# dbolya/yolact

Measured on AMD Instinct MI355X. Metric: images/sec (550x550, batch 8 per GPU), YOLACT yolact_resnet50 forward + Detect (Fast NMS), higher is better.
Workload: dtype f32 (fp32 in / fp32 accumulate / fp32 out; 92 % of the GEMM time on fp16x2 tiles = every fp32 operand as two fp16 pieces by round to nearest (22 significant bits + 2 signs: exact for ~2/3 of all fp32 values, one fp32 ulp otherwise), 3 exact piece products per product on the fp16 matrix pipe; measure

## Files before the change

### include/yolact_amd.h

```cpp
#ifndef YOLACT_AMD_H
#define YOLACT_AMD_H
#include <stddef.h>
#include <stdint.h>

#ifdef __cplusplus
extern "C" {
#endif

#define YMI_ABI_VERSION 9

#define YMI_EFORMAT (-4)
#define YMI_EUNSUPPORTED (-5)

enum { YMI_ACT_NONE = 0, YMI_ACT_RELU = 1, YMI_ACT_LEAKY01 = 2, YMI_ACT_TANH = 3, YMI_ACT_SIGMOID = 4 };
enum { YMI_RES_NONE = 0, YMI_RES_ADD = 1, YMI_RES_BILINEAR = 2 };

typedef struct {
  int32_t n0, n1;
  int32_t act;
  int32_t row_stride;
  int64_t batch_stride;
  float *ptr;
} ymi_conv_seg;

// ... 535 lines not shown
  int64_t ws_bytes;
  int32_t B, H, W, Cout, ldg, _pad0;
} ymi_stem_wgrad_desc;
int ymi_stem_wgrad_nhwc_f32(const ymi_stem_wgrad_desc *d, void *stream);

int ymi_maxpool_fwd_nhwc_f32(const float *x, float *y, int B, int H, int W, int C, void *stream);
int ymi_maxpool_bwd_nhwc_f32(const float *x, const float *dy, float *dx, int B, int H, int W, int C, void *stream);

typedef struct ymi_stem_desc {
  const float *x;
  float *y;
  int32_t B, H, W, cout_pad;
  const void *w_h2;
  const float *scale_h2, *bias;
  float *y_amax;
  int32_t kpad, _pad0;
} ymi_stem_desc;
int ymi_stem_pool_f32(const ymi_stem_desc *d, void *stream);

typedef struct ymi_chain_desc {
  const float *x, *res;
  float *y, *z;
  const void *w_a_h2, *w_b_h2;
  const float *scale_a_h2, *bias_a, *scale_b_h2, *bias_b;
  const float *x_amax;
  float *y_amax, *z_amax;
  int64_t M;
  int32_t ldx, res_ld, ldy, ldz;
  int32_t k_a, n_a, n_b;
  int32_t cout_pad_a, cout_pad_b;
  int32_t act_a, act_b, _pad0;
  const float *res_amax;
  float gain_a, bias_max_a;
} ymi_chain_desc;
int ymi_pointwise_chain_f32(const ymi_chain_desc *d, void *stream);

typedef struct ymi_stage_exit_desc {
  ymi_chain_desc chain;
  int32_t B, H, W, y_stride;
} ymi_stage_exit_desc;
int ymi_stage_exit_chain_f32(const ymi_stage_exit_desc *d, void *stream);

enum { YMI_OP_NOP = 0, YMI_OP_CONV = 1, YMI_OP_WINO = 2, YMI_OP_DCN = 3, YMI_OP_CHAIN = 4, YMI_OP_STEM = 5, YMI_OP_INPUT = 6,
       YMI_OP_BILINEAR = 7, YMI_OP_MAXPOOL = 8, YMI_OP_BILINEAR_ADD = 9, YMI_OP_RECORD = 10, YMI_OP_WAIT = 11, YMI_OP_MEMSET = 12,
       YMI_OP_STAGE_EXIT = 13 };
enum { YMI_SEC_NONE = 0, YMI_SEC_BACKBONE = 1, YMI_SEC_FPN = 2, YMI_SEC_PROTO = 3, YMI_SEC_HEADS = 4 };
typedef struct ymi_plan_op {
  int32_t kind;
  int32_t stream;
  int32_t section;
  int32_t _pad;
  const void *desc;
  void *p[3];
  int64_t i[8];
  double f[2];
} ymi_plan_op;
int ymi_event_create(void **ev);
int ymi_event_destroy(void *ev);
int ymi_plan_run(const ymi_plan_op *ops, int first, int last, void *stream_a, void *stream_b, void *const *events, int overlap,
                 int skip_sections, int32_t *failed_op);

enum {
  YMI_WS_WINO_V = 1,
  YMI_WS_WINO_M = 2,
  YMI_WS_SPLITK = 3,
  YMI_WS_MASK_IOU = 4,
// ... 78 lines not shown
```

### yolact_amd/_lib.py

```python
from __future__ import annotations

import ctypes as C
import os

_HERE = os.path.dirname(os.path.abspath(__file__))
LIB_PATH = os.path.join(_HERE, 'libyolact_amd.so')

ABI_VERSION = 9

ACT_NONE, ACT_RELU, ACT_LEAKY01, ACT_TANH, ACT_SIGMOID = 0, 1, 2, 3, 4
RES_NONE, RES_ADD, RES_BILINEAR = 0, 1, 2
TILE_AUTO, TILE_128x128, TILE_128x64, TILE_64x64, TILE_128x32, TILE_64x128 = 0, 1, 2, 3, 4, 5
TILE_32x32_K4, TILE_64x32_K2, TILE_32x64_K2 = 6, 7, 8
TILE_64x64_S3, TILE_64x64_S4, TILE_64x128_S3, TILE_128x64_S3, TILE_32x32_K4_S4, TILE_64x32_K2_S3, TILE_32x64_K2_S3 = range(9, 16)
TILE_NAMES = {1: '128x128', 2: '128x64', 3: '64x64', 4: '128x32', 5: '64x128', 6: '32x32k4', 7: '64x32k2', 8: '32x64k2',
              9: '64x64s3', 10: '64x64s4', 11: '64x128s3', 12: '128x64s3', 13: '32x32k4s4', 14: '64x32k2s3', 15: '32x64k2s3',
              16: '128x128w8', 17: '256x128w8', 18: '128x256w8', 19: '128x128s3', 20: '128x128w8s3', 21: '256x128w8s3',
              22: '128x128w8s4'}
TILE_128x128_W8, TILE_256x128_W8, TILE_128x256_W8 = 16, 17, 18
TILE_128x128_S3, TILE_128x128_W8_S3, TILE_256x128_W8_S3, TILE_128x128_W8_S4 = 19, 20, 21, 22
TILE_WG_128x256 = 23
TILE_X3 = 32
X3_BASE_TILES = (1, 2, 3, 5, 6, 7, 8, 9, 11, 12, 16, 17, 19, 20, 21, 22)
for _t in X3_BASE_TILES:
# ... 241 lines not shown
                ('out_class', C.c_void_p), ('out_coef', C.c_void_p), ('out_prior', C.c_void_p), ('out_rec', C.c_void_p)]


class DetectGreedyWs(C.Structure):
    _fields_ = [('box_scale', C.c_float), ('_pad0', C.c_int32), ('ws', C.c_void_p)]


class JpegInfo(C.Structure):
    _fields_ = [('width', C.c_int32), ('height', C.c_int32), ('ncomp', C.c_int32), ('progressive', C.c_int32),
                ('orientation', C.c_int32), ('color', C.c_int32), ('out_width', C.c_int32), ('out_height', C.c_int32),
                ('hs', C.c_int32 * 3), ('vs', C.c_int32 * 3), ('hf', C.c_int32 * 3), ('vf', C.c_int32 * 3),
                ('bw', C.c_int32 * 3), ('bh', C.c_int32 * 3), ('dw', C.c_int32 * 3), ('dh', C.c_int32 * 3),
                ('coef_count', C.c_int64), ('plane_bytes', C.c_int64)]


class JpegEncDesc(C.Structure):
    _fields_ = [('img', C.c_void_p), ('h', C.c_int32), ('w', C.c_int32), ('row_stride', C.c_int64), ('quality', C.c_int32),
                ('subsampling', C.c_int32), ('out', C.c_void_p), ('out_capacity', C.c_int64), ('out_len', C.c_void_p),
                ('ws', C.c_void_p)]


JPEG_SUB_444, JPEG_SUB_420 = 0, 2
JPEG_HEADER_BYTES = 623


class ChainDesc(C.Structure):
    _fields_ = [('x', C.c_void_p), ('res', C.c_void_p), ('y', C.c_void_p), ('z', C.c_void_p),
                ('w_a_h2', C.c_void_p), ('w_b_h2', C.c_void_p),
                ('scale_a_h2', C.c_void_p), ('bias_a', C.c_void_p), ('scale_b_h2', C.c_void_p), ('bias_b', C.c_void_p),
                ('x_amax', C.c_void_p), ('y_amax', C.c_void_p), ('z_amax', C.c_void_p),
                ('M', C.c_int64), ('ldx', C.c_int32), ('res_ld', C.c_int32), ('ldy', C.c_int32), ('ldz', C.c_int32),
                ('k_a', C.c_int32), ('n_a', C.c_int32), ('n_b', C.c_int32), ('cout_pad_a', C.c_int32), ('cout_pad_b', C.c_int32),
                ('act_a', C.c_int32), ('act_b', C.c_int32), ('_pad0', C.c_int32),
                ('res_amax', C.c_void_p), ('gain_a', C.c_float), ('bias_max_a', C.c_float)]


class StageExitDesc(C.Structure):
    _fields_ = [('chain', ChainDesc), ('B', C.c_int32), ('H', C.c_int32), ('W', C.c_int32), ('y_stride', C.c_int32)]


class StemDesc(C.Structure):
    _fields_ = [('x', C.c_void_p), ('y', C.c_void_p), ('B', C.c_int32), ('H', C.c_int32), ('W', C.c_int32), ('cout_pad', C.c_int32),
                ('w_h2', C.c_void_p), ('scale_h2', C.c_void_p), ('bias', C.c_void_p), ('y_amax', C.c_void_p),
                ('kpad', C.c_int32), ('_pad0', C.c_int32)]


class PlanOp(C.Structure):
    _fields_ = [('kind', C.c_int32), ('stream', C.c_int32), ('section', C.c_int32), ('_pad', C.c_int32), ('desc', C.c_void_p),
                ('p', C.c_void_p * 3), ('i', C.c_int64 * 8), ('f', C.c_double * 2)]


(OP_NOP, OP_CONV, OP_WINO, OP_DCN, OP_CHAIN, OP_STEM, OP_INPUT, OP_BILINEAR, OP_MAXPOOL, OP_BILINEAR_ADD, OP_RECORD, OP_WAIT,
 OP_MEMSET, OP_STAGE_EXIT) = range(14)
SEC_NONE, SEC_BACKBONE, SEC_FPN, SEC_PROTO, SEC_HEADS = range(5)


class MaskIouShape(C.Structure):
    _fields_ = [('A', C.c_int32), ('B', C.c_int32), ('n', C.c_int64)]


class ApMatchDesc(C.Structure):
    _fields_ = [('cls', C.c_void_p), ('box_score', C.c_void_p), ('mask_score', C.c_void_p), ('box_iou', C.c_void_p),
                ('mask_iou', C.c_void_p), ('crowd_box_iou', C.c_void_p), ('crowd_mask_iou', C.c_void_p), ('gt_cls', C.c_void_p),
                ('crowd_cls', C.c_void_p), ('rec_key', C.c_void_p), ('rec_score', C.c_void_p), ('rec_flags', C.c_void_p),
                ('gt_count', C.c_void_p), ('base', C.c_int64), ('cap', C.c_int64),
                ('N', C.c_int32), ('G', C.c_int32), ('Gc', C.c_int32), ('num_classes', C.c_int32)]

# ... 160 lines not shown
```

### yolact_amd/csrc/chain.hip

```cpp
#include "gemm_h2.h"
#include <type_traits>

int ymi_internal_prof_begin(double flops, int tile, int kind, hipStream_t s);
void ymi_internal_prof_end(int idx, hipStream_t s);

namespace {

using namespace ymi_h2;

typedef unsigned u32x4 __attribute__((ext_vector_type(4)));

constexpr int K1 = 64, N1 = 256, PX = 32, NW = 8;
constexpr int RS1 = 2 * K1 + 16;
constexpr int RS2 = 2 * N1 + 16;
constexpr int A1_PLANE = PX * RS1, A2_PLANE = PX * RS2;
constexpr int A1_BUF = 2 * A1_PLANE, A2_BUF = 2 * A2_PLANE;
constexpr int OFF_A1 = 0, OFF_A2 = OFF_A1 + 2 * A1_BUF, OFF_SC = OFF_A2 + 2 * A2_BUF, OFF_EP = OFF_SC + 2 * (2 * NW * 4),
              CH_LDS = OFF_EP + NW * 2 * 4 * 32;
constexpr int OFF_EP2 = CH_LDS, OFF_WL = OFF_EP2 + NW * 2 * 4 * 32, CH_LDS_X = OFF_WL + 128 * N1 * 2;
static_assert(CH_LDS_X <= 160 * 1024, "LDS of a CU");

struct ChainParams {
  const float *x, *res, *x_amax;
  const void *wa, *wb;
  const float *sa, *ba, *sb, *bb;
  float *y, *z, *y_amax, *z_amax;
  int M, ldx, res_ld, ldy, ldz, act_a, act_b;
  unsigned wa_plane, wb_plane;
};
struct ChainParamsX : ChainParams {
  unsigned long long mag_w, mag_h;
  int H, W, y_stride;
};

template <int N2>
__global__ __launch_bounds__(64 * NW) void chain_h2_k(const std::conditional_t<N2 == 128, ChainParamsX, ChainParams> p) {
#if defined(__HIP_DEVICE_COMPILE__)
  constexpr int NT = N2 / 64;
  constexpr bool EXIT = N2 == 128;
  __shared__ __attribute__((aligned(16))) char lds[EXIT ? CH_LDS_X : CH_LDS];
  const int t = threadIdx.x, lane = t & 63, wave = __builtin_amdgcn_readfirstlane(t >> 6);
  const int lr = lane & 15, g = lane >> 4;
  const int q2 = wave & 3, i2 = wave >> 2;
  float sA, invA;
  ymi_h2_scale(ymi_amax_read(p.x_amax), sA, invA);
  const ymi_amax_pre apre_y = ymi_amax_prefetch(p.y_amax);
  const ymi_amax_pre apre_z = ymi_amax_prefetch(p.z_amax);
  const bool two = p.z != nullptr;

  f16x8 w3h[2][2], w3l[2][2], w1h[NT][8], w1l[EXIT ? 1 : NT][EXIT ? 1 : 8];
#pragma unroll
  for (int j = 0; j < 2; ++j)
#pragma unroll
    for (int c = 0; c < 2; ++c) {
      const char *src = reinterpret_cast<const char *>(p.wa) + (size_t)(32 * wave + 16 * j + lr) * (2 * K1) + c * 64 + g * 16;
      w3h[j][c] = *reinterpret_cast<const f16x8 *>(src);
      w3l[j][c] = *reinterpret_cast<const f16x8 *>(src + p.wa_plane);
    }
#pragma unroll
  for (int tt = 0; tt < NT; ++tt)
#pragma unroll
    for (int c = 0; c < 8; ++c) {
      const f16x8 z8 = {0, 0, 0, 0, 0, 0, 0, 0};
      const char *src = reinterpret_cast<const char *>(p.wb) + (size_t)(16 * NT * q2 + 16 * tt + lr) * (2 * N1) + c * 64 + g * 16;
      w1h[tt][c] = two ? *reinterpret_cast<const f16x8 *>(src) : z8;
      if constexpr (!EXIT) w1l[tt][c] = two ? *reinterpret_cast<const f16x8 *>(src + p.wb_plane) : z8;
    }
  if constexpr (EXIT) {
#pragma unroll
    for (int k = 0; k < 8; ++k) {
      const int c = t >> 6;
      const char *src = reinterpret_cast<const char *>(p.wb) + p.wb_plane + (size_t)(16 * k + lr) * (2 * N1) + c * 64 + g * 16;
      const f16x8 z8 = {0, 0, 0, 0, 0, 0, 0, 0};
      *reinterpret_cast<f16x8 *>(lds + OFF_WL + ((k * 8 + c) * 64 + lane) * 16) = two ? *reinterpret_cast<const f16x8 *>(src) : z8;
    }
  }
  if (lr == 0) {
#pragma unroll
    for (int j = 0; j < 2; ++j) {
      const int n = 32 * wave + 16 * j + 4 * g;
      f32x4 sc, bi;
#pragma unroll
      for (int e = 0; e < 4; ++e) { sc[e] = p.sa[n + e] * invA; bi[e] = p.ba ? p.ba[n + e] : 0.f; }
      *reinterpret_cast<f32x4 *>(lds + OFF_EP + ((wave * 2 + j) * 4 + g) * 32) = sc;
      *reinterpret_cast<f32x4 *>(lds + OFF_EP + ((wave * 2 + j) * 4 + g) * 32 + 16) = bi;
    }
  }
  f32x4 sc1 = {1.f, 1.f, 1.f, 1.f}, bi1 = {0.f, 0.f, 0.f, 0.f};
  if constexpr (EXIT) {
    if (lr == 0) {
#pragma unroll
      for (int tt = 0; tt < NT; ++tt) {
        const int n = 16 * NT * q2 + 16 * tt + 4 * g;
        f32x4 sc = sc1, bi = bi1;
        if (two) {
#pragma unroll
          for (int e = 0; e < 4; ++e) { sc[e] = p.sb[n + e]; bi[e] = p.bb ? p.bb[n + e] : 0.f; }
        }
        *reinterpret_cast<f32x4 *>(lds + OFF_EP2 + ((wave * 2 + tt) * 4 + g) * 32) = sc;
        *reinterpret_cast<f32x4 *>(lds + OFF_EP2 + ((wave * 2 + tt) * 4 + g) * 32 + 16) = bi;
      }
    }
  } else if (two) {
#pragma unroll
    for (int e = 0; e < 4; ++e) { sc1[e] = p.sb[16 * q2 + 4 * g + e]; bi1[e] = p.bb ? p.bb[16 * q2 + 4 * g + e] : 0.f; }
  }
  const float slope_a = ymi_act_slope(p.act_a);
  const float slope_b = ymi_act_slope(p.act_b);

  const int ntiles = (p.M + PX - 1) / PX;
  const __amdgpu_buffer_rsrc_t xrs = buf_rsrc(p.x, (unsigned)p.M * (unsigned)p.ldx * 4u);
  const __amdgpu_buffer_rsrc_t rrs = buf_rsrc(p.res ? p.res : p.x, p.res ? (int)((unsigned)p.M * (unsigned)p.res_ld * 4u) : 0);
  const __amdgpu_buffer_rsrc_t yrs = buf_rsrc(p.y, (unsigned)p.M * (unsigned)p.ldy * 4u);
  const __amdgpu_buffer_rsrc_t zrs = buf_rsrc(p.z ? p.z : p.y, p.z ? (int)((unsigned)p.M * (unsigned)p.ldz * 4u) : 0);
  const int xp = t >> 4, xc = t & 15;
  auto load_x = [&](int tile) {
    const int m = tile * PX + xp;
    const unsigned off = (tile < ntiles && m < p.M) ? (unsigned)(m * p.ldx + 4 * xc) * 4u : OOB;
    return __builtin_bit_cast(f32x4, __builtin_amdgcn_raw_buffer_load_b128(xrs, off, 0, 0));
  };
  auto load_res = [&](int tile, f32x4 (&r)[2][2]) {
#pragma unroll
    for (int i = 0; i < 2; ++i) {
      const int m = tile * PX + 16 * i + lr;
      const unsigned off = (tile < ntiles && m < p.M) ? (unsigned)(m * p.res_ld + 32 * wave + 4 * g) * 4u : OOB;
#pragma unroll
      for (int j = 0; j < 2; ++j) r[i][j] = __builtin_bit_cast(f32x4, __builtin_amdgcn_raw_buffer_load_b128(rrs, off + 64u * j, 0, 0));
    }
  };

  float am_y = 0.f, am_z = 0.f;
  f32x4 xv;
  const int grid = (int)gridDim.x;
  auto iteration = [&](const int tile, auto buf_c, f32x4 (&rv)[2][2], f32x4 (&rn)[2][2]) {
    constexpr int BUF = decltype(buf_c)::value;
    char *const a1 = lds + OFF_A1 + BUF * A1_BUF;
    char *const a2w = lds + OFF_A2 + BUF * A2_BUF;
    const char *const a2r = lds + OFF_A2 + (BUF ^ 1) * A2_BUF;
    float *const scw = reinterpret_cast<float *>(lds + OFF_SC) + BUF * (2 * NW);
    const float *const scr = reinterpret_cast<const float *>(lds + OFF_SC) + (BUF ^ 1) * (2 * NW);
    {
      const f32x4 v = xv * sA;
      f16x4 h4, l4;
#pragma unroll
      for (int e = 0; e < 4; ++e) {
        const _Float16 h = (_Float16)v[e];
        h4[e] = h;
        l4[e] = (_Float16)(v[e] - (float)h);
      }
      char *dst = a1 + xp * RS1 + xc * 8;
      *reinterpret_cast<f16x4 *>(dst) = h4;
      *reinterpret_cast<f16x4 *>(dst + A1_PLANE) = l4;
    }
    xv = load_x(tile + grid);
    load_res(tile + grid, rn);
    YMI_BARRIER();
    if (two) {
      f32x4 tot[NT];
#pragma unroll
      for (int tt = 0; tt < NT; ++tt) tot[tt] = f32x4{0.f, 0.f, 0.f, 0.f};
#pragma unroll
      for (int c0 = 0; c0 < 8; c0 += 2) {
        f16x8 xh[2], xl[2];
        f32x4 a2[2][NT];
#pragma unroll
        for (int u = 0; u < 2; ++u) {
          xh[u] = *reinterpret_cast<const f16x8 *>(a2r + (16 * i2 + lr) * RS2 + (c0 + u) * 64 + g * 16);
          xl[u] = *reinterpret_cast<const f16x8 *>(a2r + A2_PLANE + (16 * i2 + lr) * RS2 + (c0 + u) * 64 + g * 16);
#pragma unroll
          for (int tt = 0; tt < NT; ++tt) a2[u][tt] = f32x4{0.f, 0.f, 0.f, 0.f};
        }
        if constexpr (EXIT) {
          f16x8 wl[2][NT];
#pragma unroll
          for (int u = 0; u < 2; ++u)
#pragma unroll
            for (int tt = 0; tt < NT; ++tt)
              wl[u][tt] = *reinterpret_cast<const f16x8 *>(lds + OFF_WL + ((((NT * q2 + tt) * 8) + c0 + u) * 64 + lane) * 16);
#pragma unroll
          for (int pr = 0; pr < 3; ++pr)
#pragma unroll
            for (int u = 0; u < 2; ++u)
#pragma unroll
              for (int tt = 0; tt < NT; ++tt)
                a2[u][tt] = ymi_mfma16(pr == 0 ? wl[u][tt] : w1h[tt][c0 + u], pr == 1 ? xl[u] : xh[u], a2[u][tt]);
        } else {
#pragma unroll
          for (int pr = 0; pr < 3; ++pr)
// ... 29 lines not shown
    f32x4 acc[2][2];
#pragma unroll
    for (int i = 0; i < 2; ++i)
#pragma unroll
      for (int j = 0; j < 2; ++j) acc[i][j] = f32x4{0.f, 0.f, 0.f, 0.f};
#pragma unroll
    for (int c = 0; c < 2; ++c) {
      f16x8 xh[2], xl[2];
#pragma unroll
      for (int i = 0; i < 2; ++i) {
        xh[i] = *reinterpret_cast<const f16x8 *>(a1 + (16 * i + lr) * RS1 + c * 64 + g * 16);
        xl[i] = *reinterpret_cast<const f16x8 *>(a1 + A1_PLANE + (16 * i + lr) * RS1 + c * 64 + g * 16);
      }
#pragma unroll
      for (int pr = 0; pr < 3; ++pr)
#pragma unroll
        for (int i = 0; i < 2; ++i)
#pragma unroll
          for (int j = 0; j < 2; ++j)
            acc[i][j] = ymi_mfma16(pr == 0 ? w3l[j][c] : w3h[j][c], pr == 1 ? xl[i] : xh[i], acc[i][j]);
    }
#pragma unroll
    for (int i = 0; i < 2; ++i) {
      const int m = tile * PX + 16 * i + lr;
      const bool ok = m < p.M;
      bool keep = ok;
      if constexpr (EXIT) {
        const unsigned r = (unsigned)(((unsigned long long)(unsigned)m * p.mag_w) >> 32);
        const unsigned w = (unsigned)m - r * (unsigned)p.W;
        const unsigned h = r - (unsigned)(((unsigned long long)r * p.mag_h) >> 32) * (unsigned)p.H;
        keep = ok && (p.y_stride == 1 || ((h | w) & 1u) == 0);
      }
      const unsigned yoff = keep ? (unsigned)(m * p.ldy + 32 * wave + 4 * g) * 4u : OOB;
      float tm = 0.f;
#pragma unroll
      for (int j = 0; j < 2; ++j) {
        const f32x4 sc3 = *reinterpret_cast<const f32x4 *>(lds + OFF_EP + ((wave * 2 + j) * 4 + g) * 32);
        const f32x4 bi3 = *reinterpret_cast<const f32x4 *>(lds + OFF_EP + ((wave * 2 + j) * 4 + g) * 32 + 16);
        f32x4 v = acc[i][j] * sc3 + bi3 + rv[i][j];
#pragma unroll
        for (int e = 0; e < 4; ++e) v[e] = fmaxf(v[e], slope_a * v[e]);
        if (!ok) v = f32x4{0.f, 0.f, 0.f, 0.f};
        acc[i][j] = v;
        tm = fmaxf(tm, ymi_absmax4(v));
        __builtin_amdgcn_raw_buffer_store_b128(__builtin_bit_cast(u32x4, v), yrs, yoff + 64u * j, 0, 0);
      }
      am_y = fmaxf(am_y, tm);
      if (two) {
        const unsigned tmb = ymi_wave_umax63(__builtin_bit_cast(unsigned, tm));
        float sT, invT;
        ymi_h2_scale(__builtin_bit_cast(float, (unsigned)__builtin_amdgcn_readlane((int)tmb, 63)), sT, invT);
#pragma unroll
        for (int j = 0; j < 2; ++j) {
          const f32x4 v = acc[i][j] * sT;
          f16x4 h4, l4;
#pragma unroll
          for (int e = 0; e < 4; ++e) {
            const _Float16 h = (_Float16)v[e];
            h4[e] = h;
            l4[e] = (_Float16)(v[e] - (float)h);
          }
          char *dst = a2w + (16 * i + lr) * RS2 + (32 * wave + 16 * j + 4 * g) * 2;
          *reinterpret_cast<f16x4 *>(dst) = h4;
          *reinterpret_cast<f16x4 *>(dst + A2_PLANE) = l4;
        }
        if (lane == 0) scw[i * NW + wave] = invT;
      }
    }
  };
  int tile = blockIdx.x;
  f32x4 ra[2][2], rb[2][2];
  xv = load_x(tile);
  load_res(tile, ra);
  for (; tile < ntiles + (two ? grid : 0); tile += 2 * grid) {
    iteration(tile, std::integral_constant<int, 0>{}, ra, rb);
    iteration(tile + grid, std::integral_constant<int, 1>{}, rb, ra);
  }
  if (p.y_amax) ymi_amax_finish(apre_y, am_y);
  if (two && p.z_amax) ymi_amax_finish(apre_z, am_z);
#endif
}

}

int ymi_internal_chain2(const ymi_chain_desc *d, hipStream_t s);

extern "C" int ymi_pointwise_chain_f32(const ymi_chain_desc *d, void *stream) {
  if (!d) return YMI_ENULL;
  if (!d->x || !d->w_a_h2 || !d->scale_a_h2 || !d->y || !d->x_amax) return YMI_ENULL;
  if (d->z && (!d->w_b_h2 || !d->scale_b_h2)) return YMI_ENULL;
  const bool wide = d->k_a == 128 || d->k_a == 256;
  if (d->M <= 0 || (!wide && (d->k_a != K1 || d->n_a != N1 || (d->z && d->n_b != 64)))) return YMI_EARG;
  if (wide && (d->n_a != 4 * d->k_a || (d->z && d->n_b != d->k_a))) return YMI_EARG;
  if (d->act_a < 0 || d->act_a > YMI_ACT_LEAKY01 || d->act_b < 0 || d->act_b > YMI_ACT_LEAKY01) return YMI_EARG;
  if (d->ldx < d->k_a || d->ldy < d->n_a || (d->z && d->ldz < d->n_b) || (d->res && d->res_ld < d->n_a)) return YMI_ESHAPE;
  if ((d->ldx | d->ldy | d->ldz | d->res_ld) & 3) return YMI_ESHAPE;
  if ((((uintptr_t)d->x) | ((uintptr_t)d->y) | ((uintptr_t)d->z) | ((uintptr_t)d->res) | ((uintptr_t)d->w_a_h2) | ((uintptr_t)d->w_b_h2)) & 15)
    return YMI_ESHAPE;
  if (d->M * (int64_t)(d->ldy > d->res_ld ? d->ldy : d->res_ld) >= (1LL << 29) || d->M * (int64_t)d->ldx >= (1LL << 29)) return YMI_ESHAPE;
  if (wide) return ymi_internal_chain2(d, (hipStream_t)stream);
  if (d->cout_pad_a < N1 || (d->z && d->cout_pad_b < 64)) return YMI_ESHAPE;
  ChainParams p;
  p.x = d->x; p.res = d->res; p.x_amax = d->x_amax; p.wa = d->w_a_h2; p.wb = d->w_b_h2;
  p.sa = d->scale_a_h2; p.ba = d->bias_a; p.sb = d->scale_b_h2; p.bb = d->bias_b;
  p.y = d->y; p.z = d->z; p.y_amax = d->y_amax; p.z_amax = d->z_amax;
  p.M = (int)d->M; p.ldx = d->ldx; p.res_ld = d->res_ld; p.ldy = d->ldy; p.ldz = d->ldz; p.act_a = d->act_a; p.act_b = d->act_b;
  p.wa_plane = (unsigned)((long)d->cout_pad_a * K1 * 2); p.wb_plane = (unsigned)((long)d->cout_pad_b * N1 * 2);
  hipStream_t s = (hipStream_t)stream;
  const int pr = ymi_internal_prof_begin(2.0 * (double)d->M * K1 * N1, YMI_TILE_H2 | YMI_TILE_64x64, 13, s);
  int dev = 0, cus = 256;
  hipGetDevice(&dev);
  hipDeviceGetAttribute(&cus, hipDeviceAttributeMultiprocessorCount, dev);
  const long ntiles = (d->M + PX - 1) / PX;
  hipLaunchKernelGGL(chain_h2_k<64>, dim3((unsigned)(ntiles < cus ? ntiles : cus)), dim3(64 * NW), 0, s, p);
  const int rc = ymi_launch_status();
  ymi_internal_prof_end(pr, s);
  if (rc == YMI_OK && d->z) {
    const int p2 = ymi_internal_prof_begin(2.0 * (double)d->M * N1 * 64, YMI_TILE_H2 | YMI_TILE_64x64, 12, s);
    ymi_internal_prof_end(p2, s);
  }
  return rc;
}

extern "C" int ymi_stage_exit_chain_f32(const ymi_stage_exit_desc *e, void *stream) {
  if (!e) return YMI_ENULL;
  const ymi_chain_desc *d = &e->chain;
  if (!d->x || !d->w_a_h2 || !d->scale_a_h2 || !d->y || !d->x_amax || !d->z || !d->w_b_h2 || !d->scale_b_h2) return YMI_ENULL;
  if (d->k_a != K1 || d->n_a != N1 || d->n_b != 128 || (e->y_stride != 1 && e->y_stride != 2)) return YMI_EARG;
  if (d->M <= 0 || e->B <= 0 || e->H <= 0 || e->W <= 0 || d->M != (int64_t)e->B * e->H * e->W) return YMI_EARG;
  if (d->act_a < 0 || d->act_a > YMI_ACT_LEAKY01 || d->act_b < 0 || d->act_b > YMI_ACT_LEAKY01) return YMI_EARG;
  if (d->ldx < K1 || d->ldy < N1 || d->ldz < 128 || (d->res && d->res_ld < N1)) return YMI_ESHAPE;
  if ((d->ldx | d->ldy | d->ldz | d->res_ld) & 3) return YMI_ESHAPE;
  if ((((uintptr_t)d->x) | ((uintptr_t)d->y) | ((uintptr_t)d->z) | ((uintptr_t)d->res) | ((uintptr_t)d->w_a_h2) | ((uintptr_t)d->w_b_h2)) & 15)
    return YMI_ESHAPE;
  const int64_t ldmax = d->ldy > d->res_ld ? (d->ldy > d->ldz ? d->ldy : d->ldz) : (d->res_ld > d->ldz ? d->res_ld : d->ldz);
  if (d->M * ldmax >= (1LL << 29) || d->M * (int64_t)d->ldx >= (1LL << 29)) return YMI_ESHAPE;
  if (d->cout_pad_a < N1 || d->cout_pad_b < 128) return YMI_ESHAPE;
  if (d->M * (int64_t)(e->H > e->W ? e->H : e->W) >= (1LL << 32)) return YMI_ESHAPE;
  ChainParamsX p;
  p.x = d->x; p.res = d->res; p.x_amax = d->x_amax; p.wa = d->w_a_h2; p.wb = d->w_b_h2;
  p.sa = d->scale_a_h2; p.ba = d->bias_a; p.sb = d->scale_b_h2; p.bb = d->bias_b;
  p.y = d->y; p.z = d->z; p.y_amax = d->y_amax; p.z_amax = d->z_amax;
  p.M = (int)d->M; p.ldx = d->ldx; p.res_ld = d->res_ld; p.ldy = d->ldy; p.ldz = d->ldz; p.act_a = d->act_a; p.act_b = d->act_b;
  p.wa_plane = (unsigned)((long)d->cout_pad_a * K1 * 2); p.wb_plane = (unsigned)((long)d->cout_pad_b * N1 * 2);
  p.H = e->H; p.W = e->W; p.y_stride = e->y_stride;
  p.mag_w = ((1ULL << 32) + (unsigned)e->W - 1) / (unsigned)e->W;
  p.mag_h = ((1ULL << 32) + (unsigned)e->H - 1) / (unsigned)e->H;
  hipStream_t s = (hipStream_t)stream;
  const int pr = ymi_internal_prof_begin(2.0 * (double)d->M * K1 * N1, YMI_TILE_H2 | YMI_TILE_64x64, 13, s);
  int dev = 0, cus = 256;
  hipGetDevice(&dev);
  hipDeviceGetAttribute(&cus, hipDeviceAttributeMultiprocessorCount, dev);
  const long ntiles = (d->M + PX - 1) / PX;
  hipLaunchKernelGGL(chain_h2_k<128>, dim3((unsigned)(ntiles < cus ? ntiles : cus)), dim3(64 * NW), 0, s, p);
  const int rc = ymi_launch_status();
  ymi_internal_prof_end(pr, s);
  if (rc == YMI_OK) {
    const int p2 = ymi_internal_prof_begin(2.0 * (double)d->M * N1 * 128, YMI_TILE_H2 | YMI_TILE_64x64, 12, s);
    ymi_internal_prof_end(p2, s);
  }
  return rc;
// ... 2 lines not shown
```

### yolact_amd/plan_tune.py

```python
from __future__ import annotations

import ctypes as C
import os

import torch

from . import _lib as L
from . import tune_table as TT


def _ceil(a, b):
    return (a + b - 1) // b * b


def _desc_pointers(d):
    out = []
    if isinstance(d, C.Array):
        for e in d:
            out += _desc_pointers(e) if isinstance(e, (C.Structure, C.Array)) else ([int(e)] if isinstance(e, int) and e else [])
        return out
    for f in d._fields_:
        name, typ = f[0], f[1]
        v = getattr(d, name)
        if typ is C.c_void_p:
# ... 64 lines not shown
                disk.update(TT.read_table_file(cache_path))
        n0 = len(disk)
        self.run(x)
        s = L.stream_ptr()
        e0, e1 = torch.cuda.Event(enable_timing=True), torch.cuda.Event(enable_timing=True)
        measure = mode != 'table'
        self._tune_direct(e0, e1, s, reps, disk, measure)
        self._tune_winograd(e0, e1, s, reps, disk, measure)
        self._fuse_pointwise_chains(e0, e1, s, reps, disk, measure)
        torch.cuda.synchronize(self.device)
        if cache_path and (len(disk) != n0 or mode == 'force'):
            TT.write_table_file(cache_path, disk, self.device)
        self.tune_entries = disk
        return self.tune_table

    def _splitk_ws(self, where, numel):
        ws = self._sk_ws.get(where)
        if ws is None or ws.numel() < numel:
            ws = self._sk_ws[where] = torch.empty(numel, dtype=torch.float32, device=self.device)
            for fn, dptr, _n, w in self.ops:
                if fn is self.lib.ymi_conv2d_nhwc_f32 and w == where and dptr.contents.split_k > 1:
                    dptr.contents.split_ws = ws.data_ptr()
                elif fn is self.lib.ymi_dcn_v2_forward_f32 and w == where and dptr.contents.conv.split_k > 1:
                    dptr.contents.conv.split_ws = ws.data_ptr()
        return ws

    @staticmethod
    def _splitk_ok(d):
        return (d.kh == 1 and d.kw == 1 and d.pad == 0 and d.Cin == d.Kpad and d.Cin % 32 == 0 and d.nseg == 1
                and d.Cout % 4 == 0 and d.seg[0].act <= L.ACT_LEAKY01 and d.res_mode in (L.RES_NONE, L.RES_ADD)
                and d.B * d.Ho * d.Wo <= 16384 and d.Kpad >= 256)

    def _fuse_pointwise_chains(self, e0, e1, s, reps, disk, measure):
        self.chain_table, self.chainx_table = [], []
        if not self.h2 or os.environ.get('YOLACT_AMD_CHAIN', '1') != '1':
            return
        lib = self.lib

        def timed(run):
            return _timed(run, e0, e1, reps)
        self._fuse_stage_exit(s, disk, measure, timed)
        i = 0
        while i < len(self.ops):
            f3, p3, n3, w3 = self.ops[i]
            i += 1
            if f3 is not lib.ymi_conv2d_nhwc_f32 or (i - 1) in self.wide_ops:
                continue
            d3 = p3.contents
            M = d3.B * d3.Ho * d3.Wo
            P_ = d3.Cin
            if not ((d3.kh, d3.kw, d3.stride, d3.pad, d3.nseg) == (1, 1, 1, 0, 1) and P_ in (64, 128, 256) and d3.Cout == 4 * P_
                    and d3.res_mode == L.RES_ADD and not d3.res_after_act and d3.seg[0].n0 == 0 and d3.seg[0].act <= L.ACT_LEAKY01
                    and d3.w_h2 and d3.x_amax and M * max(d3.seg[0].row_stride, d3.res_ld) < (1 << 29)):
                continue
            if P_ > 64 and os.environ.get('YOLACT_AMD_CHAIN2', '0') not in ('1', 'force'):
                continue
            pair = False
            if i < len(self.ops) and self.ops[i][0] is lib.ymi_conv2d_nhwc_f32 and self.ops[i][3] == w3 and i not in self.wide_ops:
                d1 = self.ops[i][1].contents
                pair = ((d1.kh, d1.kw, d1.stride, d1.pad, d1.Cin, d1.Cout, d1.nseg) == (1, 1, 1, 0, 4 * P_, P_, 1)
                        and d1.res_mode == L.RES_NONE and d1.x == d3.seg[0].ptr and d1.ldx == d3.seg[0].row_stride
                        and d1.seg[0].n0 == 0 and d1.seg[0].act <= L.ACT_LEAKY01 and bool(d1.w_h2))
            if P_ > 64 and not pair:
                continue
            cd = _fill_chain(L.ChainDesc(), d3, d1 if pair else None)
            if P_ > 64:
                info = getattr(self, '_desc_info', {}).get(C.addressof(d3))
                if info is None or info[1] is None:
                    continue
                cd.gain_a, cd.bias_max_a = info[0].l1_gain()
                cd.res_amax = self._slot_ptr(info[1])
            name = n3
            if pair:
                f1, p1, n1, w1 = self.ops[i]
                name = n3 + '+' + n1
                in_place = int(cd.z) == int(cd.x) and cd.ldz == cd.ldx
                if (_rows_overlap(M, cd.z, cd.ldz, cd.y, cd.ldy) or _rows_overlap(M, cd.z, cd.ldz, cd.res, cd.res_ld)
                        or (_rows_overlap(M, cd.z, cd.ldz, cd.x, cd.ldx) and not in_place)):
                    continue
            cptr = C.pointer(cd)
            key = TT.chain_key('chain' if pair else 'chain1', d3.B, d3.Ho, d3.Wo, P_ if P_ > 64 else None, self.mode)
            ent = disk.get(key)
            if P_ > 64 and os.environ.get('YOLACT_AMD_CHAIN2') == 'force':
                ent = [1, 0.0, 0.0]
            if ent is None:
                self.tune_misses += 1
                if not measure or lib.ymi_pointwise_chain_f32(cptr, s) != 0:
                    continue
                t_plan = timed((lambda: (f3(p3, s), f1(p1, s))) if pair else (lambda: f3(p3, s)))
                t_one = timed(lambda: lib.ymi_pointwise_chain_f32(cptr, s))
                ent = disk[key] = [1 if t_one < 0.97 * t_plan else 0, round(t_plan, 4), round(t_one, 4)]
            self.chain_table.append((name, ent[0], ent[1], ent[2]))
            if ent[0] and lib.ymi_pointwise_chain_f32(cptr, s) == 0:
                self.keepalive.append(cd)
                self.ops[i - 1] = (lib.ymi_pointwise_chain_f32, cptr, name, w3)
                if pair:
                    self.ops[i] = ('nop', None, n1 + '[fused into ' + n3 + ']', w1)
                    i += 1

    def stage_exit_candidates(self):
        conv = self.lib.ymi_conv2d_nhwc_f32
        selected = {int(p) for li, p in getattr(self, '_stage_out_ptr', {}).items() if li in self.net.backbone_selected}
        out = []
        for i3, (f3, p3, n3, w3) in enumerate(self.ops):
            if f3 is not conv or i3 in self.wide_ops:
                continue
            d3 = p3.contents
            if not ((d3.kh, d3.kw, d3.stride, d3.pad, d3.nseg, d3.Cin, d3.Cout) == (1, 1, 1, 0, 1, 64, 256)
                    and d3.res_mode == L.RES_ADD and not d3.res_after_act and d3.seg[0].n0 == 0 and d3.seg[0].act <= L.ACT_LEAKY01):
                continue
            yptr, ldy = int(d3.seg[0].ptr or 0), d3.seg[0].row_stride
            if not yptr or yptr in selected:
                continue
            i1 = None
            for j in range(i3 + 1, len(self.ops)):
                fj, pj, _, wj = self.ops[j]
                if wj != w3 or fj in ('record', 'nop'):
                    continue
                if fj is conv and j not in self.wide_ops:
                    d1 = pj.contents
                    if ((d1.kh, d1.kw, d1.stride, d1.pad, d1.Cin, d1.Cout, d1.nseg) == (1, 1, 1, 0, 256, 128, 1)
                            and d1.res_mode == L.RES_NONE and int(d1.x or 0) == yptr and d1.ldx == ldy
                            and (d1.B, d1.H, d1.W) == (d3.B, d3.Ho, d3.Wo) and d1.seg[0].n0 == 0 and d1.seg[0].act <= L.ACT_LEAKY01):
                        i1 = j
                break
            if i1 is None:
                continue
            downs, ok = [], True
            for j in range(i3 + 1, len(self.ops)):
                fj, pj, _, _ = self.ops[j]
                if j == i1 or isinstance(fj, str) or self.sections[j] != 'backbone':
                    continue
                if fj is conv:
                    dj = pj.contents
                    if (int(dj.x or 0) == yptr and (dj.kh, dj.kw, dj.stride, dj.pad) == (1, 1, 2, 0) and dj.nseg == 1
                            and (dj.B, dj.H, dj.W, dj.ldx) == (d3.B, d3.Ho, d3.Wo, ldy) and int(dj.res or 0) != yptr
                            and int(dj.seg[0].ptr or 0) != yptr):
                        downs.append(j)
                        continue
                    ptrs = _desc_pointers(dj)
                elif isinstance(pj, tuple):
                    ptrs = [a for a in pj if isinstance(a, int)]
                else:
                    ptrs = _desc_pointers(pj.contents)
                if yptr in ptrs:
                    ok = False
                    break
            if ok:
                out.append((i3, i1, downs))
        return out

    def _fuse_stage_exit(self, s, disk, measure, timed):
        mode = os.environ.get('YOLACT_AMD_CHAIN_EXIT', '1')
        self.chainx_table = []
        if mode not in ('1', 'force'):
            return
        lib = self.lib
        for i3, i1, downs in self.stage_exit_candidates():
            f3, p3, n3, w3 = self.ops[i3]
            f1, p1, n1, w1 = self.ops[i1]
            d3, d1 = p3.contents, p1.contents
            if not (d3.w_h2 and d3.x_amax and d1.w_h2):
                continue
            M = d3.B * d3.Ho * d3.Wo
            if M * max(d3.seg[0].row_stride, d3.res_ld, d1.seg[0].row_stride) >= (1 << 29):
                continue
            xd = L.StageExitDesc()
            cd = _fill_chain(xd.chain, d3, d1)
            xd.B, xd.H, xd.W = d3.B, d3.Ho, d3.Wo
            xd.y_stride = 2 if downs else 1
            if (_rows_overlap(M, cd.z, cd.ldz, cd.y, cd.ldy) or _rows_overlap(M, cd.z, cd.ldz, cd.x, cd.ldx)
                    or (cd.res and _rows_overlap(M, cd.z, cd.ldz, cd.res, cd.res_ld))):
                continue
            xptr = C.pointer(xd)
            name = n3 + '+' + n1
            key = TT.chainx_key(d3.B, d3.Ho, d3.Wo, self.mode)
            ent = disk.get(key)
            if mode == 'force':
                ent = [1, 0.0, 0.0]
            if ent is None:
                self.tune_misses += 1
                if not measure or lib.ymi_stage_exit_chain_f32(xptr, s) != 0:
                    continue
# ... 308 lines not shown
```

Measured before the change: 2360.

## Fuse downsample shortcut 1x1 conv into the bottleneck pointwise chain kernel

Adds an ENTRY variant of the pointwise chain kernel. It computes the projection shortcut 1x1 conv (64->256) from the block input in-kernel with fp16x2 MFMA and adds it as the residual, instead of reading a residual tensor produced by a separate conv launch. The planner finds matching shortcut convs, times fused against unfused, and replaces the shortcut op with a nop when the fused form wins. This removes one kernel launch and the write and re-read of the 256-channel shortcut tensor per first-block-of-stage. It costs extra LDS, registers and MFMA work in the chain kernel.

```diff
diff --git a/include/yolact_amd.h b/include/yolact_amd.h
--- a/include/yolact_amd.h
+++ b/include/yolact_amd.h
@@ -591,6 +591,10 @@
   int32_t act_a, act_b, _pad0;
   const float *res_amax;
   float gain_a, bias_max_a;
+  const float *x0, *x0_amax;
+  const void *w_d_h2;
+  const float *scale_d_h2, *bias_d;
+  int32_t ldx0, cout_pad_d;
 } ymi_chain_desc;
 int ymi_pointwise_chain_f32(const ymi_chain_desc *d, void *stream);
 
diff --git a/yolact_amd/_lib.py b/yolact_amd/_lib.py
--- a/yolact_amd/_lib.py
+++ b/yolact_amd/_lib.py
@@ -297,7 +297,9 @@
                 ('M', C.c_int64), ('ldx', C.c_int32), ('res_ld', C.c_int32), ('ldy', C.c_int32), ('ldz', C.c_int32),
                 ('k_a', C.c_int32), ('n_a', C.c_int32), ('n_b', C.c_int32), ('cout_pad_a', C.c_int32), ('cout_pad_b', C.c_int32),
                 ('act_a', C.c_int32), ('act_b', C.c_int32), ('_pad0', C.c_int32),
-                ('res_amax', C.c_void_p), ('gain_a', C.c_float), ('bias_max_a', C.c_float)]
+                ('res_amax', C.c_void_p), ('gain_a', C.c_float), ('bias_max_a', C.c_float),
+                ('x0', C.c_void_p), ('x0_amax', C.c_void_p), ('w_d_h2', C.c_void_p), ('scale_d_h2', C.c_void_p),
+                ('bias_d', C.c_void_p), ('ldx0', C.c_int32), ('cout_pad_d', C.c_int32)]
 
 
 class StageExitDesc(C.Structure):
diff --git a/yolact_amd/csrc/chain.hip b/yolact_amd/csrc/chain.hip
--- a/yolact_amd/csrc/chain.hip
+++ b/yolact_amd/csrc/chain.hip
@@ -19,6 +19,8 @@
               CH_LDS = OFF_EP + NW * 2 * 4 * 32;
 constexpr int OFF_EP2 = CH_LDS, OFF_WL = OFF_EP2 + NW * 2 * 4 * 32, CH_LDS_X = OFF_WL + 128 * N1 * 2;
 static_assert(CH_LDS_X <= 160 * 1024, "LDS of a CU");
+constexpr int OFF_A0 = CH_LDS, OFF_EPD = OFF_A0 + 2 * A1_BUF, OFF_WDL = OFF_EPD + NW * 2 * 4 * 32, CH_LDS_E = OFF_WDL + N1 * K1 * 2;
+static_assert(CH_LDS_E <= 160 * 1024, "LDS of a CU");
 
 struct ChainParams {
   const float *x, *res, *x_amax;
@@ -32,18 +34,30 @@
   unsigned long long mag_w, mag_h;
   int H, W, y_stride;
 };
-
-template <int N2>
-__global__ __launch_bounds__(64 * NW) void chain_h2_k(const std::conditional_t<N2 == 128, ChainParamsX, ChainParams> p) {
+struct ChainParamsE : ChainParams {
+  const float *x0, *x0_amax;
+  const void *wd;
+  const float *sd, *bd;
+  int ldx0;
+  unsigned wd_plane;
+};
+template <int N2, bool ENTRY>
+using chain_params_t = std::conditional_t<ENTRY, ChainParamsE, std::conditional_t<N2 == 128, ChainParamsX, ChainParams>>;
+
+template <int N2, bool ENTRY = false>
+__global__ __launch_bounds__(64 * NW) void chain_h2_k(const chain_params_t<N2, ENTRY> p) {
 #if defined(__HIP_DEVICE_COMPILE__)
   constexpr int NT = N2 / 64;
   constexpr bool EXIT = N2 == 128;
-  __shared__ __attribute__((aligned(16))) char lds[EXIT ? CH_LDS_X : CH_LDS];
+  static_assert(!(ENTRY && EXIT), "the entry form is the 64-wide pair's");
+  __shared__ __attribute__((aligned(16))) char lds[EXIT ? CH_LDS_X : ENTRY ? CH_LDS_E : CH_LDS];
   const int t = threadIdx.x, lane = t & 63, wave = __builtin_amdgcn_readfirstlane(t >> 6);
   const int lr = lane & 15, g = lane >> 4;
   const int q2 = wave & 3, i2 = wave >> 2;
   float sA, invA;
   ymi_h2_scale(ymi_amax_read(p.x_amax), sA, invA);
+  float sD = 1.f, invD = 1.f;
+  if constexpr (ENTRY) ymi_h2_scale(ymi_amax_read(p.x0_amax), sD, invD);
   const ymi_amax_pre apre_y = ymi_amax_prefetch(p.y_amax);
   const ymi_amax_pre apre_z = ymi_amax_prefetch(p.z_amax);
   const bool two = p.z != nullptr;
@@ -57,6 +71,17 @@
       w3h[j][c] = *reinterpret_cast<const f16x8 *>(src);
       w3l[j][c] = *reinterpret_cast<const f16x8 *>(src + p.wa_plane);
     }
+  f16x8 wdh[ENTRY ? 2 : 1][ENTRY ? 2 : 1];
+  if constexpr (ENTRY) {
+#pragma unroll
+    for (int j = 0; j < 2; ++j)
+#pragma unroll
+      for (int c = 0; c < 2; ++c) {
+        const char *src = reinterpret_cast<const char *>(p.wd) + (size_t)(32 * wave + 16 * j + lr) * (2 * K1) + c * 64 + g * 16;
+        wdh[j][c] = *reinterpret_cast<const f16x8 *>(src);
+        *reinterpret_cast<f16x8 *>(lds + OFF_WDL + (((wave * 2 + j) * 2 + c) * 64 + lane) * 16) = *reinterpret_cast<const f16x8 *>(src + p.wd_plane);
+      }
+  }
 #pragma unroll
   for (int tt = 0; tt < NT; ++tt)
 #pragma unroll
@@ -84,6 +109,12 @@
       for (int e = 0; e < 4; ++e) { sc[e] = p.sa[n + e] * invA; bi[e] = p.ba ? p.ba[n + e] : 0.f; }
       *reinterpret_cast<f32x4 *>(lds + OFF_EP + ((wave * 2 + j) * 4 + g) * 32) = sc;
       *reinterpret_cast<f32x4 *>(lds + OFF_EP + ((wave * 2 + j) * 4 + g) * 32 + 16) = bi;
+      if constexpr (ENTRY) {
+#pragma unroll
+        for (int e = 0; e < 4; ++e) { sc[e] = p.sd[n + e] * invD; bi[e] = p.bd ? p.bd[n + e] : 0.f; }
+        *reinterpret_cast<f32x4 *>(lds + OFF_EPD + ((wave * 2 + j) * 4 + g) * 32) = sc;
+        *reinterpret_cast<f32x4 *>(lds + OFF_EPD + ((wave * 2 + j) * 4 + g) * 32 + 16) = bi;
+      }
     }
   }
   f32x4 sc1 = {1.f, 1.f, 1.f, 1.f}, bi1 = {0.f, 0.f, 0.f, 0.f};
@@ -119,6 +150,17 @@
     const unsigned off = (tile < ntiles && m < p.M) ? (unsigned)(m * p.ldx + 4 * xc) * 4u : OOB;
     return __builtin_bit_cast(f32x4, __builtin_amdgcn_raw_buffer_load_b128(xrs, off, 0, 0));
   };
+  __amdgpu_buffer_rsrc_t x0rs = xrs;
+  if constexpr (ENTRY) x0rs = buf_rsrc(p.x0, (unsigned)p.M * (unsigned)p.ldx0 * 4u);
+  auto load_x0 = [&](int tile) {
+    if constexpr (ENTRY) {
+      const int m = tile * PX + xp;
+      const unsigned off = (tile < ntiles && m < p.M) ? (unsigned)(m * p.ldx0 + 4 * xc) * 4u : OOB;
+      return __builtin_bit_cast(f32x4, __builtin_amdgcn_raw_buffer_load_b128(x0rs, off, 0, 0));
+    } else {
+      return f32x4{0.f, 0.f, 0.f, 0.f};
+    }
+  };
   auto load_res = [&](int tile, f32x4 (&r)[2][2]) {
 #pragma unroll
     for (int i = 0; i < 2; ++i) {
@@ -130,11 +172,12 @@
   };
 
   float am_y = 0.f, am_z = 0.f;
-  f32x4 xv;
+  f32x4 xv, x0v;
   const int grid = (int)gridDim.x;
   auto iteration = [&](const int tile, auto buf_c, f32x4 (&rv)[2][2], f32x4 (&rn)[2][2]) {
     constexpr int BUF = decltype(buf_c)::value;
     char *const a1 = lds + OFF_A1 + BUF * A1_BUF;
+    char *const a0 = lds + OFF_A0 + BUF * A1_BUF;
     char *const a2w = lds + OFF_A2 + BUF * A2_BUF;
     const char *const a2r = lds + OFF_A2 + (BUF ^ 1) * A2_BUF;
     float *const scw = reinterpret_cast<float *>(lds + OFF_SC) + BUF * (2 * NW);
@@ -152,8 +195,22 @@
       *reinterpret_cast<f16x4 *>(dst) = h4;
       *reinterpret_cast<f16x4 *>(dst + A1_PLANE) = l4;
     }
+    if constexpr (ENTRY) {
+      const f32x4 v = x0v * sD;
+      f16x4 h4, l4;
+#pragma unroll
+      for (int e = 0; e < 4; ++e) {
+        const _Float16 h = (_Float16)v[e];
+        h4[e] = h;
+        l4[e] = (_Float16)(v[e] - (float)h);
+      }
+      char *dst = a0 + xp * RS1 + xc * 8;
+      *reinterpret_cast<f16x4 *>(dst) = h4;
+      *reinterpret_cast<f16x4 *>(dst + A1_PLANE) = l4;
+    }
     xv = load_x(tile + grid);
-    load_res(tile + grid, rn);
+    if constexpr (ENTRY) x0v = load_x0(tile + grid);
+    else load_res(tile + grid, rn);
     YMI_BARRIER();
     if (two) {
       f32x4 tot[NT];
@@ -249,12 +306,38 @@
         keep = ok && (p.y_stride == 1 || ((h | w) & 1u) == 0);
       }
       const unsigned yoff = keep ? (unsigned)(m * p.ldy + 32 * wave + 4 * g) * 4u : OOB;
+      f32x4 accd[2];
+      if constexpr (ENTRY) {
+#pragma unroll
+        for (int j = 0; j < 2; ++j) accd[j] = f32x4{0.f, 0.f, 0.f, 0.f};
+#pragma unroll
+        for (int c = 0; c < 2; ++c) {
+          f16x8 wdl[2];
+#pragma unroll
+          for (int j = 0; j < 2; ++j) wdl[j] = *reinterpret_cast<const f16x8 *>(lds + OFF_WDL + (((wave * 2 + j) * 2 + c) * 64 + lane) * 16);
+          const f16x8 xh = *reinterpret_cast<const f16x8 *>(a0 + (16 * i + lr) * RS1 + c * 64 + g * 16);
+          const f16x8 xl = *reinterpret_cast<const f16x8 *>(a0 + A1_PLANE + (16 * i + lr) * RS1 + c * 64 + g * 16);
+#pragma unroll
+          for (int pr = 0; pr < 3; ++pr)
+#pragma unroll
+            for (int j = 0; j < 2; ++j)
+              accd[j] = ymi_mfma16(pr == 0 ? wdl[j] : wdh[j][c], pr == 1 ? xl : xh, accd[j]);
+        }
+      }
       float tm = 0.f;
 #pragma unroll
       for (int j = 0; j < 2; ++j) {
         const f32x4 sc3 = *reinterpret_cast<const f32x4 *>(lds + OFF_EP + ((wave * 2 + j) * 4 + g) * 32);
         const f32x4 bi3 = *reinterpret_cast<const f32x4 *>(lds + OFF_EP + ((wave * 2 + j) * 4 + g) * 32 + 16);
-        f32x4 v = acc[i][j] * sc3 + bi3 + rv[i][j];
+        f32x4 v;
+        if constexpr (ENTRY) {
+          const f32x4 scd = *reinterpret_cast<const f32x4 *>(lds + OFF_EPD + ((wave * 2 + j) * 4 + g) * 32);
+          const f32x4 bid = *reinterpret_cast<const f32x4 *>(lds + OFF_EPD + ((wave * 2 + j) * 4 + g) * 32 + 16);
+          const f32x4 r = accd[j] * scd + bid;
+          v = acc[i][j] * sc3 + bi3 + r;
+        } else {
+          v = acc[i][j] * sc3 + bi3 + rv[i][j];
+        }
 #pragma unroll
         for (int e = 0; e < 4; ++e) v[e] = fmaxf(v[e], slope_a * v[e]);
         if (!ok) v = f32x4{0.f, 0.f, 0.f, 0.f};
@@ -288,7 +371,8 @@
   int tile = blockIdx.x;
   f32x4 ra[2][2], rb[2][2];
   xv = load_x(tile);
-  load_res(tile, ra);
+  if constexpr (ENTRY) x0v = load_x0(tile);
+  else load_res(tile, ra);
   for (; tile < ntiles + (two ? grid : 0); tile += 2 * grid) {
     iteration(tile, std::integral_constant<int, 0>{}, ra, rb);
     iteration(tile + grid, std::integral_constant<int, 1>{}, rb, ra);
@@ -315,9 +399,18 @@
   if ((((uintptr_t)d->x) | ((uintptr_t)d->y) | ((uintptr_t)d->z) | ((uintptr_t)d->res) | ((uintptr_t)d->w_a_h2) | ((uintptr_t)d->w_b_h2)) & 15)
     return YMI_ESHAPE;
   if (d->M * (int64_t)(d->ldy > d->res_ld ? d->ldy : d->res_ld) >= (1LL << 29) || d->M * (int64_t)d->ldx >= (1LL << 29)) return YMI_ESHAPE;
+  const bool entry = d->x0 != nullptr;
+  if (entry) {
+    if (wide || d->res || d->k_a != K1 || d->n_a != N1) return YMI_EARG;
+    if (!d->w_d_h2 || !d->scale_d_h2 || !d->x0_amax) return YMI_ENULL;
+    if (d->ldx0 < K1 || (d->ldx0 & 3) || ((((uintptr_t)d->x0) | ((uintptr_t)d->w_d_h2)) & 15)) return YMI_ESHAPE;
+    if (d->M * (int64_t)d->ldx0 >= (1LL << 29) || d->cout_pad_d < N1) return YMI_ESHAPE;
+  }
   if (wide) return ymi_internal_chain2(d, (hipStream_t)stream);
   if (d->cout_pad_a < N1 || (d->z && d->cout_pad_b < 64)) return YMI_ESHAPE;
-  ChainParams p;
+  ChainParamsE p;
+  p.x0 = d->x0; p.x0_amax = d->x0_amax; p.wd = d->w_d_h2; p.sd = d->scale_d_h2; p.bd = d->bias_d; p.ldx0 = d->ldx0;
+  p.wd_plane = (unsigned)((long)d->cout_pad_d * K1 * 2);
   p.x = d->x; p.res = d->res; p.x_amax = d->x_amax; p.wa = d->w_a_h2; p.wb = d->w_b_h2;
   p.sa = d->scale_a_h2; p.ba = d->bias_a; p.sb = d->scale_b_h2; p.bb = d->bias_b;
   p.y = d->y; p.z = d->z; p.y_amax = d->y_amax; p.z_amax = d->z_amax;
@@ -329,9 +422,15 @@
   hipGetDevice(&dev);
   hipDeviceGetAttribute(&cus, hipDeviceAttributeMultiprocessorCount, dev);
   const long ntiles = (d->M + PX - 1) / PX;
-  hipLaunchKernelGGL(chain_h2_k<64>, dim3((unsigned)(ntiles < cus ? ntiles : cus)), dim3(64 * NW), 0, s, p);
+  const dim3 grid((unsigned)(ntiles < cus ? ntiles : cus));
+  if (entry) hipLaunchKernelGGL((chain_h2_k<64, true>), grid, dim3(64 * NW), 0, s, p);
+  else hipLaunchKernelGGL(chain_h2_k<64>, grid, dim3(64 * NW), 0, s, static_cast<const ChainParams &>(p));
   const int rc = ymi_launch_status();
   ymi_internal_prof_end(pr, s);
+  if (rc == YMI_OK && entry) {
+    const int pd = ymi_internal_prof_begin(2.0 * (double)d->M * K1 * N1, YMI_TILE_H2 | YMI_TILE_64x64, 12, s);
+    ymi_internal_prof_end(pd, s);
+  }
   if (rc == YMI_OK && d->z) {
     const int p2 = ymi_internal_prof_begin(2.0 * (double)d->M * N1 * 64, YMI_TILE_H2 | YMI_TILE_64x64, 12, s);
     ymi_internal_prof_end(p2, s);
@@ -344,6 +443,7 @@
   const ymi_chain_desc *d = &e->chain;
   if (!d->x || !d->w_a_h2 || !d->scale_a_h2 || !d->y || !d->x_amax || !d->z || !d->w_b_h2 || !d->scale_b_h2) return YMI_ENULL;
   if (d->k_a != K1 || d->n_a != N1 || d->n_b != 128 || (e->y_stride != 1 && e->y_stride != 2)) return YMI_EARG;
+  if (d->x0) return YMI_EARG;
   if (d->M <= 0 || e->B <= 0 || e->H <= 0 || e->W <= 0 || d->M != (int64_t)e->B * e->H * e->W) return YMI_EARG;
   if (d->act_a < 0 || d->act_a > YMI_ACT_LEAKY01 || d->act_b < 0 || d->act_b > YMI_ACT_LEAKY01) return YMI_EARG;
   if (d->ldx < K1 || d->ldy < N1 || d->ldz < 128 || (d->res && d->res_ld < N1)) return YMI_ESHAPE;
diff --git a/yolact_amd/plan_tune.py b/yolact_amd/plan_tune.py
--- a/yolact_amd/plan_tune.py
+++ b/yolact_amd/plan_tune.py
@@ -120,13 +120,15 @@
                 and d.B * d.Ho * d.Wo <= 16384 and d.Kpad >= 256)
 
     def _fuse_pointwise_chains(self, e0, e1, s, reps, disk, measure):
-        self.chain_table, self.chainx_table = [], []
+        self.chain_table, self.chainx_table, self.chaine_table = [], [], []
         if not self.h2 or os.environ.get('YOLACT_AMD_CHAIN', '1') != '1':
             return
         lib = self.lib
 
         def timed(run):
             return _timed(run, e0, e1, reps)
+        entry_mode = os.environ.get('YOLACT_AMD_CHAIN_ENTRY', '1')
+        entry = {i3: idn for idn, i3, _ in self.entry_chain_candidates()} if entry_mode in ('1', 'force') else {}
         self._fuse_stage_exit(s, disk, measure, timed)
         i = 0
         while i < len(self.ops):
@@ -185,6 +187,39 @@
                 if pair:
                     self.ops[i] = ('nop', None, n1 + '[fused into ' + n3 + ']', w1)
                     i += 1
+                    if P_ == 64 and (i - 2) in entry:
+                        self._fuse_entry_shortcut(i - 2, entry[i - 2], cd, s, disk, measure, timed, entry_mode)
+
+    def _fuse_entry_shortcut(self, ic, idn, cd, s, disk, measure, timed, mode):
+        lib = self.lib
+        fd, pd, nd, wd = self.ops[idn]
+        ce = self._entry_chain_desc(cd, idn)
+        if ce is None:
+            return
+        dd = pd.contents
+        eptr, cptr = C.pointer(ce), C.pointer(cd)
+        key = TT.chain_key('chain', dd.B, dd.Ho, dd.Wo, 64, self.mode)
+        ent = disk.get(key)
+        if mode == 'force':
+            ent = [1, 0.0, 0.0]
+        if ent is None:
+            self.tune_misses += 1
+            if not measure or lib.ymi_pointwise_chain_f32(eptr, s) != 0:
+                return
+            t_plan = timed(lambda: (fd(pd, s), lib.ymi_pointwise_chain_f32(cptr, s)))
+            t_one = timed(lambda: lib.ymi_pointwise_chain_f32(eptr, s))
+            ent = disk[key] = [1 if t_one < 0.97 * t_plan else 0, round(t_plan, 4), round(t_one, 4)]
+        fc, _, nc, wc = self.ops[ic]
+        self.chaine_table.append((nc, ent[0], ent[1], ent[2]))
+        if ent[0] and lib.ymi_pointwise_chain_f32(eptr, s) == 0:
+            self.keepalive.append(ce)
+            self.ops[ic] = (fc, eptr, nc, wc)
+            self.ops[idn] = ('nop', None, nd + '[fused into ' + nc.split('+')[0] + ']', wd)
+            names = [n for n, _ in self.conv_meta]
+            n3 = nc.split('+')[0]
+            if nd in names and n3 in names:
+                m = self.conv_meta.pop(names.index(nd))
+                self.conv_meta.insert([n for n, _ in self.conv_meta].index(n3) + 1, m)
 
     def stage_exit_candidates(self):
         conv = self.lib.ymi_conv2d_nhwc_f32
@@ -237,6 +272,77 @@
             if ok:
                 out.append((i3, i1, downs))
         return out
+
+    def entry_chain_candidates(self):
+        conv = self.lib.ymi_conv2d_nhwc_f32
+        out = []
+        for i3, (f3, p3, _, w3) in enumerate(self.ops):
+            if f3 is not conv or i3 in self.wide_ops or i3 + 1 >= len(self.ops):
+                continue
+            d3 = p3.contents
+            if not ((d3.kh, d3.kw, d3.stride, d3.pad, d3.nseg, d3.Cin, d3.Cout) == (1, 1, 1, 0, 1, 64, 256)
+                    and d3.res_mode == L.RES_ADD and not d3.res_after_act and d3.seg[0].n0 == 0 and d3.seg[0].act <= L.ACT_LEAKY01
+                    and d3.res):
+                continue
+            f1, p1, _, w1 = self.ops[i3 + 1]
+            if f1 is not conv or w1 != w3 or (i3 + 1) in self.wide_ops:
+                continue
+            d1 = p1.contents
+            if not ((d1.kh, d1.kw, d1.stride, d1.pad, d1.Cin, d1.Cout, d1.nseg) == (1, 1, 1, 0, 256, 64, 1)
+                    and d1.res_mode == L.RES_NONE and d1.x == d3.seg[0].ptr and d1.ldx == d3.seg[0].row_stride
+                    and d1.seg[0].n0 == 0 and d1.seg[0].act <= L.ACT_LEAKY01):
+                continue
+            rptr = int(d3.res)
+            idn = None
+            for j in range(i3 - 1, -1, -1):
+                fj, pj, _, _ = self.ops[j]
+                if fj is conv and any(int(pj.contents.seg[k].ptr or 0) == rptr for k in range(pj.contents.nseg)):
+                    idn = j
+                    break
+            if idn is None or idn in self.wide_ops:
+                continue
+            dd = self.ops[idn][1].contents
+            if not ((dd.kh, dd.kw, dd.stride, dd.pad, dd.nseg, dd.Cin, dd.Cout) == (1, 1, 1, 0, 1, 64, 256)
+                    and dd.res_mode == L.RES_NONE and dd.seg[0].act == L.ACT_NONE and dd.seg[0].n0 == 0
+                    and (dd.B, dd.Ho, dd.Wo) == (d3.B, d3.Ho, d3.Wo) and dd.seg[0].row_stride == d3.res_ld
+                    and int(dd.x or 0) != rptr):
+                continue
+            ok = True
+            for j in range(idn + 1, len(self.ops)):
+                fj, pj, _, _ = self.ops[j]
+                if j == i3 or isinstance(fj, str):
+                    continue
+                if isinstance(pj, tuple):
+                    ptrs = [a for a in pj if isinstance(a, int)]
+                else:
+                    ptrs = _desc_pointers(pj.contents)
+                if rptr not in ptrs:
+                    continue
+                if fj is conv:
+                    dj = pj.contents
+                    n_out = sum(1 for k in range(dj.nseg) if int(dj.seg[k].ptr or 0) == rptr)
+                    ok = ptrs.count(rptr) == n_out
+                else:
+                    ok = False
+                break
+            if ok:
+                out.append((idn, i3, i3 + 1))
+        return out
+
+    def _entry_chain_desc(self, cd, idn):
+        dd = self.ops[idn][1].contents
+        if not (dd.w_h2 and dd.scale_h2 and dd.x_amax and dd.x):
+            return None
+        ce = L.ChainDesc.from_buffer_copy(cd)
+        ce.res, ce.res_ld = None, 0
+        ce.x0, ce.ldx0, ce.x0_amax = dd.x, dd.ldx, dd.x_amax
+        ce.w_d_h2, ce.scale_d_h2, ce.bias_d, ce.cout_pad_d = dd.w_h2, dd.scale_h2, dd.bias, _ceil(dd.Cout, 128)
+        M = int(ce.M)
+        if M * ce.ldx0 >= (1 << 29) or _rows_overlap(M, ce.y, ce.ldy, ce.x0, ce.ldx0):
+            return None
+        if _rows_overlap(M, ce.z, ce.ldz, ce.x0, ce.ldx0) and not (int(ce.z) == int(ce.x0) and ce.ldz == ce.ldx0):
+            return None
+        return ce
 
     def _fuse_stage_exit(self, s, disk, measure, timed):
         mode = os.environ.get('YOLACT_AMD_CHAIN_EXIT', '1')
```

Result: faster. 2397, median of 6 (+1.5%).
